# locuslab/lcp-physics

Measured on NVIDIA H100. Metric: LCP solves/sec (LCPFunction fwd+bwd, batch=4096 x 64 contacts, fp32), higher is better.
Workload: dtype f32 I/O and iterates; the condensed n x n KKT matrix is formed, factored and solved in f64

## Files before the change

lcp_physics_b200/csrc/lcp_condensed.cuh:

```cuda
#pragma once
#include "lcp_device.cuh"

namespace lcpb200 {
namespace cnd {

constexpr int NT = 256;
constexpr int UC = 8;
constexpr int CSMAX = 6;
constexpr int KS = 8;
constexpr int LMAX = 16;
constexpr int STATUS_UNSUPPORTED = -100;

struct CPlan {
  int ok;
  int n, m, e, N, NP, NS;
  int pcap;
  int wcap;
  int smem_bytes;
  int ctas_per_sm;
  int flags;
  int sbytes;
  int o_K, o_W, o_scr, o_bx, o_rdiag, o_Fd, o_Gd, o_As, o_x, o_rx, o_dx, o_qd, o_y, o_ry, o_dy,
      o_s, o_z, o_d, o_rz, o_ds, o_dz, o_rs2, o_red, o_rows, o_posof, o_clist, o_ccols, o_ncols, o_clcnt, o_misc;
};

__host__ __device__ inline size_t al16(size_t x) { return (x + 15) & ~(size_t)15; }
__host__ __device__ inline size_t scratch_bytes(int n, int m, int tsize) {
  return al16((size_t)2 * KS * m * 2) + al16((size_t)2 * KS * m * tsize) + al16((size_t)5 * m * 4) +
         al16((size_t)CSMAX * m * 2) + al16((size_t)8 * m * 4) + al16((size_t)LMAX * n * 2) + al16((size_t)n * 4) + 64;
}

inline size_t carve_plan(CPlan& P, int tsize) {
  size_t o = 0;
  const int n = P.n, m = P.m, e = P.e, NP = P.NP, pcap = P.pcap, wcap = P.wcap;
#define CND_TAKE(field, bytes) do { P.field = (int)o; o += al16((size_t)(bytes)); } while (0)
  size_t kb = (size_t)NP * NP * 8;
  if (scratch_bytes(n, m, tsize) > kb) kb = scratch_bytes(n, m, tsize);
  if ((size_t)8 * NP * 8 > kb) kb = (size_t)8 * NP * 8;
  { const size_t qn = (NP + 31) / 32, sl = (size_t)(NP / qn) * qn * qn * 32 * 8; if (sl > kb) kb = sl; }
  CND_TAKE(o_K, kb);
  CND_TAKE(o_W, (size_t)wcap * 8);
  CND_TAKE(o_scr, (size_t)pcap * 8);
  CND_TAKE(o_bx, (size_t)NP * 8);
  CND_TAKE(o_rdiag, (size_t)NP * 8);
  CND_TAKE(o_Fd, (size_t)wcap * tsize);
  CND_TAKE(o_Gd, (size_t)UC * pcap * tsize);
  CND_TAKE(o_As, (size_t)e * n * tsize);
  CND_TAKE(o_x, n * tsize); CND_TAKE(o_rx, n * tsize); CND_TAKE(o_dx, n * tsize); CND_TAKE(o_qd, n * tsize);
  CND_TAKE(o_y, e * tsize); CND_TAKE(o_ry, e * tsize); CND_TAKE(o_dy, e * tsize);
  CND_TAKE(o_s, m * tsize); CND_TAKE(o_z, m * tsize); CND_TAKE(o_d, m * tsize); CND_TAKE(o_rz, m * tsize);
  CND_TAKE(o_ds, m * tsize); CND_TAKE(o_dz, m * tsize); CND_TAKE(o_rs2, m * tsize);
  CND_TAKE(o_red, 192 * tsize);
  CND_TAKE(o_rows, pcap * 2);
  CND_TAKE(o_posof, m * 2);
  CND_TAKE(o_clist, LMAX * n * 2);
  CND_TAKE(o_ccols, UC * pcap);
  CND_TAKE(o_ncols, pcap);
  CND_TAKE(o_clcnt, n);
  CND_TAKE(o_misc, 16 * 4);
#undef CND_TAKE
  P.sbytes = 16 + (P.o_x - P.o_Fd) + (P.o_y - P.o_qd) + (P.o_misc - P.o_rows);
  return o;
}

extern __shared__ __align__(16) unsigned char cnd_smem[];

template <typename T>
struct CSmem {
  const CPlan& P;
  __device__ __forceinline__ explicit CSmem(const CPlan& p) : P(p) {}
#define CND_ACC(name, type) __device__ __forceinline__ type* name() const { return reinterpret_cast<type*>(cnd_smem + P.o_##name); }
  CND_ACC(K, double) CND_ACC(W, double) CND_ACC(scr, double) CND_ACC(bx, double) CND_ACC(rdiag, double)
  CND_ACC(Fd, T) CND_ACC(Gd, T) CND_ACC(As, T)
  CND_ACC(x, T) CND_ACC(rx, T) CND_ACC(dx, T) CND_ACC(qd, T) CND_ACC(y, T) CND_ACC(ry, T) CND_ACC(dy, T)
  CND_ACC(s, T) CND_ACC(z, T) CND_ACC(d, T) CND_ACC(rz, T) CND_ACC(ds, T) CND_ACC(dz, T) CND_ACC(rs2, T)
  CND_ACC(red, T)
  CND_ACC(rows, unsigned short) CND_ACC(posof, unsigned short) CND_ACC(clist, unsigned short)
  CND_ACC(ccols, unsigned char) CND_ACC(ncols, unsigned char) CND_ACC(clcnt, unsigned char)
  CND_ACC(misc, int)
#undef CND_ACC
};

struct Struct {
  int ncomp, cs;
  int sh;
  int m;
};

enum { CPH_STRUCT = 0, CPH_WINV, CPH_ASSEMBLE, CPH_LU, CPH_SOLVE_RHS, CPH_SOLVE_TRI, CPH_SOLVE_POST, CPH_RESID,
       CPH_STEP, CPH_GRADS, CPH_COUNT };
template <bool ON>
struct Prof {
  long long* p;
// ... 281 lines not shown
  T* ps = e_.p_s + (size_t)sc * n;
  T* hs = e_.h_s + (size_t)sc * P.m;
  int bad = 0;
  for (int j = tid; j < n; j += NT) {
    const int body = j / 3;
    const T q = (j - 3 * body == 0) ? inertia[body] : mass[body];
    S.qd()[j] = q;
    if (!(q != T(0) && isfinite((double)q))) bad |= 2;
    ps[j] = e_.mode == 0 ? q * v[j] + e_.dt * e_.fext[(size_t)sc * n + j] : T(0);
    cl_cnt[j] = 0;
  }
  for (int t = tid; t < e * n; t += NT) S.As()[t] = A[t];
  st.ncomp = nc; st.cs = cs; st.m = m;
  st.sh = 0;
  while ((1 << st.sh) < nc) ++st.sh;
  for (int t = tid; t < UC * pcap; t += NT) { S.Gd()[t] = T(0); S.ccols()[t] = 0; }
  for (int t = tid; t < nc * cs * cs; t += NT) S.Fd()[t] = T(0);
  __syncthreads();
  for (int c = tid; c < nc; c += NT) {
    const int b1 = tb1[c], b2 = tb2[c];
    if (b1 == b2 || b1 < 0 || b2 < 0 || b1 >= nb || b2 >= nb) { bad |= 1; continue; }
    const int lo = min(b1, b2), hi = max(b1, b2);
    const int o1 = b1 < b2 ? 0 : 3, o2 = 3 - o1;
#pragma unroll
    for (int q = 0; q < 3; ++q) {
      S.ccols()[q * pcap + c] = (unsigned char)(3 * lo + q);
      S.ccols()[(3 + q) * pcap + c] = (unsigned char)(3 * hi + q);
    }
    S.ncols()[c] = 6;
    const T nx = normal[2 * c], ny = normal[2 * c + 1];
    const T p1x = p1[2 * c], p1y = p1[2 * c + 1], p2x = p2[2 * c], p2y = p2[2 * c + 1];
    T r1[3], r2[3];
    contact_row<T>(p1x, p1y, p2x, p2y, nx, ny, r1, r2);
    const T jv = r1[0] * v[3 * b1] + r1[1] * v[3 * b1 + 1] + r1[2] * v[3 * b1 + 2] +
                 r2[0] * v[3 * b2] + r2[1] * v[3 * b2 + 1] + r2[2] * v[3 * b2 + 2];
    const T rc = e_.rest[(size_t)sc * ncs + c];
#pragma unroll
    for (int q = 0; q < 3; ++q) { S.Gd()[(size_t)(o1 + q) * pcap + c] = r1[q]; S.Gd()[(size_t)(o2 + q) * pcap + c] = r2[q]; }
    S.rows()[c] = (unsigned short)c;
    S.posof()[c] = (unsigned short)c;
    if (e_.mode == 0) {
      hs[c] = jv * rc;
      contact_row<T>(p1x, p1y, p2x, p2y, ny, -nx, r1, r2);
#pragma unroll
      for (int q = 0; q < 3; ++q) {
        S.Gd()[(size_t)(o1 + q) * pcap + nc + c] = r1[q];      S.Gd()[(size_t)(o2 + q) * pcap + nc + c] = r2[q];
        S.Gd()[(size_t)(o1 + q) * pcap + 2 * nc + c] = -r1[q]; S.Gd()[(size_t)(o2 + q) * pcap + 2 * nc + c] = -r2[q];
      }
      const int rw[4] = {c, nc + 2 * c, nc + 2 * c + 1, 3 * nc + c};
#pragma unroll
      for (int r = 0; r < 4; ++r) { S.rows()[r * nc + c] = (unsigned short)rw[r]; S.posof()[rw[r]] = (unsigned short)(r * nc + c); }
      hs[nc + 2 * c] = T(0); hs[nc + 2 * c + 1] = T(0); hs[3 * nc + c] = T(0);
      S.Fd()[(size_t)(1 * 4 + 3) * nc + c] = T(1);
      S.Fd()[(size_t)(2 * 4 + 3) * nc + c] = T(1);
      S.Fd()[(size_t)(3 * 4 + 0) * nc + c] = e_.mu[(size_t)sc * ncs + c];
      S.Fd()[(size_t)(3 * 4 + 1) * nc + c] = T(-1);
      S.Fd()[(size_t)(3 * 4 + 2) * nc + c] = T(-1);
    } else {
      hs[c] = jv + jv * -rc;
    }
    for (int q = 0; q < 6; ++q) {
      const int a = q < 3 ? 3 * lo + q : 3 * hi + q - 3;
      const int slot = atomicAdd(&cl_cnt[a], 1);
      if (slot < LMAX) cl_tmp[slot * n + a] = (unsigned short)(c * 8 + q); else bad |= 1;
    }
  }
  const int anybad = __syncthreads_or(bad);
  if (anybad & 2) { *singular = 1; return false; }
  if (anybad & 1) return false;
  for (int t = tid; t < n * LMAX; t += NT) {
    const int a = t % n, l = t / n, cnt = cl_cnt[a];
    if (l < cnt) {
      const int val = cl_tmp[l * n + a];
      int rank = 0;
      for (int u = 0; u < cnt; ++u) rank += (cl_tmp[u * n + a] < val);
      S.clist()[rank * n + a] = (unsigned short)val;
    }
    if (l == 0) S.clcnt()[a] = (unsigned char)cnt;
  }
  __syncthreads();
  return true;
}

__device__ __forceinline__ double rcp64_fast(double x) {
  double r;
  asm("rcp.approx.ftz.f64 %0, %1;" : "=d"(r) : "d"(x));
  const double ax = fabs(x);
  if (!(ax > 1e-290 && ax < 1e290)) return 1.0 / x;
  r = fma(r, fma(-x, r, 1.0), r);
  r = fma(r, fma(-x, r, 1.0), r);
  return r;
}

template <typename T, int CS>
__device__ __forceinline__ void comp_inverse(const CPlan& P, CSmem<T>& S, const Struct& st) {
  const int nc_ = st.ncomp;
  for (int c = threadIdx.x; c < nc_; c += NT) {
    double M[CS][CS];
#pragma unroll
    for (int r = 0; r < CS; ++r) {
      const int i = S.rows()[r * nc_ + c];
#pragma unroll
      for (int q = 0; q < CS; ++q) M[r][q] = (double)S.Fd()[(size_t)(r * CS + q) * nc_ + c];
      M[r][r] += (i == 0xFFFF) ? 1.0 : ((P.flags & 1) ? 1.0 / (double)S.d()[i] : (double)(T(1) / S.d()[i]));
    }
    unsigned swaps = 0;
    int bit = 0;
#pragma unroll
    for (int k = 0; k < CS; ++k) {
#pragma unroll
      for (int i = k + 1; i < CS; ++i) {
        const bool sw = fabs(M[i][k]) > fabs(M[k][k]);
        swaps |= (sw ? 1u : 0u) << bit;
        ++bit;
#pragma unroll
        for (int q = 0; q < CS; ++q) { const double u = M[k][q], w = M[i][q]; M[k][q] = sw ? w : u; M[i][q] = sw ? u : w; }
      }
      const double r = rcp64_fast(M[k][k]);
      M[k][k] = 1.0;
#pragma unroll
      for (int q = 0; q < CS; ++q) M[k][q] *= r;
#pragma unroll
      for (int i = 0; i < CS; ++i) {
        if (i == k) continue;
        const double f = M[i][k];
        M[i][k] = 0.0;
#pragma unroll
        for (int q = 0; q < CS; ++q) M[i][q] = fma(-f, M[k][q], M[i][q]);
      }
    }
#pragma unroll
    for (int k = CS - 1; k >= 0; --k) {
#pragma unroll
      for (int i = CS - 1; i > k; --i) {
        --bit;
        const bool sw = (swaps >> bit) & 1u;
#pragma unroll
        for (int q = 0; q < CS; ++q) { const double u = M[q][k], w = M[q][i]; M[q][k] = sw ? w : u; M[q][i] = sw ? u : w; }
      }
    }
#pragma unroll
    for (int r = 0; r < CS; ++r)
#pragma unroll
      for (int q = 0; q < CS; ++q) S.W()[(size_t)(r * CS + q) * nc_ + c] = M[r][q];
  }
}

template <typename T, int CS>
__device__ __forceinline__ void comp_apply(CSmem<T>& S, const Struct& st, bool trans = false) {
  const int nc_ = st.ncomp;
  const int npos = nc_ * CS;
  const int sh = st.sh, cmask = (1 << sh) - 1, tot = CS << sh;
  double val[4];
#pragma unroll
  for (int u = 0; u < 4; ++u) {
    const int t = threadIdx.x + u * NT, r = t >> sh, c = t & cmask;
    val[u] = 0.0;
    if (t < tot && c < nc_) {
      double a = 0.0;
#pragma unroll
      for (int q = 0; q < CS; ++q) a = fma(S.W()[(size_t)(trans ? (q * CS + r) : (r * CS + q)) * nc_ + c], S.scr()[q * nc_ + c], a);
      val[u] = a;
    }
  }
  __syncthreads();
#pragma unroll
  for (int u = 0; u < 4; ++u) {
    const int t = threadIdx.x + u * NT, r = t >> sh, c = t & cmask;
    if (t < tot && c < nc_) S.scr()[r * nc_ + c] = val[u];
  }
  (void)npos;
}

template <typename T, int NS, int CS>
__device__ __forceinline__ void assemble_K(const CPlan& P, CSmem<T>& S, const Struct& st) {
  const int nc_ = st.ncomp;
  constexpr int NP = 16 * NS;
  const int n = P.n, N = P.N, e = P.e, tid = threadIdx.x, pcap = P.pcap;
  double* K = S.K();
  {
    double2* K2 = reinterpret_cast<double2*>(K);
    for (int t = tid; t < NP * NP / 2; t += NT) K2[t] = make_double2(0.0, 0.0);
  }
  __syncthreads();
  for (int i = tid; i < NP; i += NT) K[(size_t)i * NP + i] = i < n ? (double)S.qd()[i] : (i < N ? 0.0 : 1.0);
  for (int t = tid; t < e * n; t += NT) {
    const int k = t / n, i = t - k * n;
    const double v = (double)S.As()[t];
    K[(size_t)(n + k) * NP + i] = v;
    K[(size_t)i * NP + n + k] = v;
  }
  __syncthreads();
  const int grp = tid >> 3, q2 = tid & 7;
  for (int a0 = 0; a0 < n; a0 += NT / 8) {
    const int a = a0 + grp;
    const int cnt = a < n ? (int)S.clcnt()[a] : 0;
    int mx = cnt;
    mx = max(mx, __shfl_xor_sync(FULL, mx, 8));
    mx = max(mx, __shfl_xor_sync(FULL, mx, 16));
    for (int l = 0; l < mx; ++l) {
      if (l < cnt) {
        const int cp = S.clist()[l * n + a], c = cp >> 3, p = cp & 7;
        if (q2 < (int)S.ncols()[c]) {
          double acc = 0.0;
#pragma unroll
          for (int q = 0; q < CS; ++q) {
            double u = 0.0;
#pragma unroll
            for (int r = 0; r < CS; ++r)
              u = fma((double)S.Gd()[(size_t)p * pcap + r * nc_ + c], S.W()[(size_t)(r * CS + q) * nc_ + c], u);
            acc = fma(u, (double)S.Gd()[(size_t)q2 * pcap + q * nc_ + c], acc);
          }
          K[(size_t)S.ccols()[q2 * pcap + c] * NP + a] += acc;
        }
      }
      __syncwarp();
    }
  }
  __syncthreads();
}

template <int NS, int B0>
__device__ __forceinline__ void lu_phase(double (&a)[NS][NS], int o_buf, int o_rdiag, int& step, int ti, int tj) {
  constexpr int NP = 16 * NS;
  constexpr int L = NS - B0;
  constexpr int CW = (L <= 4) ? L : 3;
  double* const rdiag = reinterpret_cast<double*>(cnd_smem + o_rdiag);
#pragma unroll 1
  for (int kk = 0; kk < 16; kk += 2) {
    const int k = 16 * B0 + kk;
    double2* const U2 = reinterpret_cast<double2*>(cnd_smem + o_buf) + (size_t)(step & 1) * 2 * NP;
    double2* const C2 = U2 + NP;
    ++step;
    {
      const int sr = ti - kk, sc = tj - kk;
      if ((unsigned)sr < 2u) {
        double* dst = reinterpret_cast<double*>(U2) + sr;
#pragma unroll
        for (int c = B0; c < NS; ++c) dst[2 * (16 * c + tj)] = a[B0][c];
      }
      if ((unsigned)sc < 2u) {
        double* dst = reinterpret_cast<double*>(C2) + sc;
#pragma unroll
        for (int r = B0; r < NS; ++r) dst[2 * (16 * r + ti)] = a[r][B0];
      }
    }
    __syncthreads();
    const double2 pk = U2[k], pk1 = U2[k + 1];
    const double p01 = pk1.x;
    const double r0 = rcp64_fast(pk.x);
    const double r1 = pk.x * rcp64_fast(fma(pk.x, pk1.y, -(pk.y * p01)));
    const double l10 = pk.y * r0;
    if ((ti | tj) == 0) { rdiag[k] = r0; rdiag[k + 1] = r1; }
#pragma unroll
    for (int cg = B0; cg < NS; cg += CW) {
      double w0[CW], w1[CW];
#pragma unroll
      for (int q = 0; q < CW; ++q) {
        const int c = cg + q;
        if (c < NS) {
          const double2 u = U2[16 * c + tj];
          const double x1 = fma(-l10, u.x, u.y);
          w0[q] = (c == B0 && !(tj > kk)) ? 0.0 : u.x;
          w1[q] = (c == B0 && !(tj > kk + 1)) ? 0.0 : x1;
        }
      }
#pragma unroll
      for (int r = B0; r < NS; ++r) {
        const double2 cc = C2[16 * r + ti];
        double m0 = cc.x * r0;
        double m1 = fma(-m0, p01, cc.y) * r1;
        if (r == B0) {
          m0 = (ti > kk) ? m0 : 0.0;
          m1 = (ti > kk + 1) ? m1 : 0.0;
        }
#pragma unroll
        for (int q = 0; q < CW; ++q) {
          const int c = cg + q;
          if (c < NS) a[r][c] = fma(-m1, w1[q], fma(-m0, w0[q], a[r][c]));
        }
      }
    }
  }
}

template <int NS, int B0>
struct LuPhases {
  static __device__ __forceinline__ void run(double (&a)[NS][NS], int o_buf, int o_rdiag, int& step, int ti, int tj) {
    lu_phase<NS, B0>(a, o_buf, o_rdiag, step, ti, tj);
    LuPhases<NS, B0 + 1>::run(a, o_buf, o_rdiag, step, ti, tj);
  }
};
template <int NS>
struct LuPhases<NS, NS> {
  static __device__ __forceinline__ void run(double (&)[NS][NS], int, int, int&, int, int) {}
};

template <int NS> struct SolveLayout {
  static constexpr int NP = 16 * NS;
  static constexpr int QN = (NP + 31) / 32;
  static constexpr int ROUNDS = NP / QN;
  static constexpr size_t BYTES = (size_t)ROUNDS * QN * QN * 32 * 8;
};

template <int NS>
__device__ __noinline__ void factor_K(int o_K, int o_rdiag, bool trans) {
  constexpr int NP = 16 * NS, QN = SolveLayout<NS>::QN;
  int tid_;
  asm volatile("mov.u32 %0, %%tid.x;" : "=r"(tid_));
  const int ti = tid_ & 15, tj = tid_ >> 4;
  double* const K = reinterpret_cast<double*>(cnd_smem + o_K);
  double* const rdiag = reinterpret_cast<double*>(cnd_smem + o_rdiag);
  double a[NS][NS];
#pragma unroll
  for (int c = 0; c < NS; ++c)
#pragma unroll
    for (int r = 0; r < NS; ++r) a[r][c] = K[(size_t)(16 * c + tj) * NP + 16 * r + ti];
  __syncthreads();
  int step = 0;
  LuPhases<NS, 0>::run(a, o_K, o_rdiag, step, ti, tj);
  __syncthreads();
  int rowpart[NS];
  double rrow[NS];
#pragma unroll
  for (int r = 0; r < NS; ++r) {
    const int i = 16 * r + ti;
    rowpart[r] = trans ? (i / QN) * QN * QN * 32 + (i % QN) * 32 : (i % QN) * QN * 32 + i / QN;
    rrow[r] = rdiag[i];
  }
#pragma unroll
  for (int c = 0; c < NS; ++c) {
    const int j = 16 * c + tj;
    const double rj = rdiag[j];
    const int colpart = trans ? (j % QN) * QN * 32 + j / QN : (j / QN) * QN * QN * 32 + (j % QN) * 32;
#pragma unroll
    for (int r = 0; r < NS; ++r) {
      const int i = 16 * r + ti;
      K[colpart + rowpart[r]] = (i != j) ? a[r][c] * (trans ? rrow[r] : rj) : a[r][c];
    }
  }
  __syncthreads();
}

template <int QN>
struct SolveCoef {
  double dg[QN * QN];
  double rw[QN * QN];
};

template <int QN>
__device__ __forceinline__ void solve_load(SolveCoef<QN>& c, const double* blk, int r, int lane) {
#pragma unroll
  for (int t = 0; t < QN * QN; ++t) { c.dg[t] = blk[t * 32 + r]; c.rw[t] = blk[t * 32 + lane]; }
}

template <int QN>
__device__ __forceinline__ void solve_round_fwd(double (&y)[QN], const SolveCoef<QN>& c, int r, int lane) {
  double v[QN];
#pragma unroll
  for (int q = 0; q < QN; ++q) v[q] = __shfl_sync(FULL, y[q], r);
#pragma unroll
  for (int q = 0; q < QN; ++q)
#pragma unroll
    for (int qp = q + 1; qp < QN; ++qp) v[qp] = fma(-c.dg[qp * QN + q], v[q], v[qp]);
  const bool below = lane > r, own = lane == r;
#pragma unroll
  for (int qp = 0; qp < QN; ++qp) {
    double t = y[qp];
#pragma unroll
    for (int q = 0; q < QN; ++q) t = fma(-c.rw[qp * QN + q], v[q], t);
    y[qp] = below ? t : (own ? v[qp] : y[qp]);
  }
}

template <int QN>
__device__ __forceinline__ void solve_round_bwd(double (&y)[QN], const SolveCoef<QN>& c, int r, int lane) {
  double v[QN];
#pragma unroll
  for (int q = 0; q < QN; ++q) v[q] = __shfl_sync(FULL, y[q], r);
#pragma unroll
  for (int q = QN - 1; q >= 0; --q)
#pragma unroll
    for (int qp = q - 1; qp >= 0; --qp) v[qp] = fma(-c.dg[qp * QN + q], v[q], v[qp]);
  const bool above = lane < r, own = lane == r;
#pragma unroll
  for (int qp = 0; qp < QN; ++qp) {
    double t = y[qp];
#pragma unroll
    for (int q = QN - 1; q >= 0; --q) t = fma(-c.rw[qp * QN + q], v[q], t);
    y[qp] = above ? t : (own ? v[qp] : y[qp]);
  }
}

template <int NS>
__device__ __noinline__ void solve_warp(int o_K, int o_rdiag, int o_bx) {
  constexpr int NP = 16 * NS, QN = SolveLayout<NS>::QN, ROUNDS = SolveLayout<NS>::ROUNDS;
  constexpr int STRIDE = QN * QN * 32;
  static_assert(ROUNDS % 2 == 0, "the software pipeline handles two rounds per trip");
  const int lane = threadIdx.x & 31;
  const double* const S = reinterpret_cast<const double*>(cnd_smem + o_K);
  const double* const rdiag = reinterpret_cast<const double*>(cnd_smem + o_rdiag);
  double* const bx = reinterpret_cast<double*>(cnd_smem + o_bx);
  double y[QN];
#pragma unroll
  for (int q = 0; q < QN; ++q) y[q] = (QN * lane + q < NP) ? bx[QN * lane + q] : 0.0;
  SolveCoef<QN> c0, c1;
  solve_load<QN>(c0, S, 0, lane);
#pragma unroll 1
  for (int r = 0; r < ROUNDS; r += 2) {
    solve_load<QN>(c1, S + (size_t)(r + 1) * STRIDE, r + 1, lane);
    solve_round_fwd<QN>(y, c0, r, lane);
    const int rn = (r + 2 < ROUNDS) ? r + 2 : ROUNDS - 1;
    solve_load<QN>(c0, S + (size_t)rn * STRIDE, rn, lane);
    solve_round_fwd<QN>(y, c1, r + 1, lane);
  }
#pragma unroll 1
  for (int r = ROUNDS - 1; r > 0; r -= 2) {
    solve_load<QN>(c1, S + (size_t)(r - 1) * STRIDE, r - 1, lane);
    solve_round_bwd<QN>(y, c0, r, lane);
    const int rn = (r - 2 >= 0) ? r - 2 : 0;
    solve_load<QN>(c0, S + (size_t)rn * STRIDE, rn, lane);
    solve_round_bwd<QN>(y, c1, r - 1, lane);
  }
#pragma unroll
  for (int q = 0; q < QN; ++q) {
    const int i = QN * lane + q;
    if (i < NP) bx[i] = y[q] * rdiag[i];
  }
}

template <typename T, int CS, int NS, typename PF>
__device__ __noinline__ void solve_kkt(const CPlan& P, CSmem<T> S, Struct st, PF& pf, const T* rx,
                                       const T* rs, const T* rz, const T* ry, T* dx, T* ds, T* dz, T* dy,
                                       bool trans = false) {
  const int nc_ = st.ncomp;
  const int n = P.n, e = P.e, N = P.N, NP = P.NP, tid = threadIdx.x, pcap = P.pcap;
  const int npos = st.ncomp * CS;
  for (int p = tid; p < npos; p += NT) {
    const int i = S.rows()[p];
    double t = 0.0;
    if (i != 0xFFFF) t = (P.flags & 2) ? ((double)(rz ? rz[i] : T(0)) - (double)rs[i] / (double)S.d()[i]) : (double)((rz ? rz[i] : T(0)) - rs[i] / S.d()[i]);
    S.scr()[p] = t;
  }
  __syncthreads();
  comp_apply<T, CS>(S, st, trans);
  __syncthreads();
  for (int a = tid; a < NP; a += NT) {
    double acc = 0.0;
    if (a < n) {
      const int cnt = S.clcnt()[a];
      for (int l = 0; l < cnt; ++l) {
        const int cp = S.clist()[l * n + a], c = cp >> 3, p = cp & 7;
#pragma unroll
        for (int r = 0; r < CS; ++r) acc = fma((double)S.Gd()[(size_t)p * pcap + r * nc_ + c], S.scr()[r * nc_ + c], acc);
      }
      acc = -(double)(rx ? rx[a] : T(0)) - acc;
    } else if (a < N) {
      acc = -(double)(ry ? ry[a - n] : T(0));
    }
    S.bx()[a] = acc;
  }
  __syncthreads();
  pf.lap(CPH_SOLVE_RHS);
  if (tid < 32) solve_warp<NS>(P.o_K, P.o_rdiag, P.o_bx);
  __syncthreads();
  pf.lap(CPH_SOLVE_TRI);
  for (int tt = tid; tt < (CS << st.sh); tt += NT) {
    const int c = tt & ((1 << st.sh) - 1);
    if (c >= nc_) continue;
    const int p = (tt >> st.sh) * nc_ + c;
    const int i = S.rows()[p];
    double t = 0.0;
    if (i != 0xFFFF) {
      const int nc = S.ncols()[c];
      t = (P.flags & 2) ? ((double)(rz ? rz[i] : T(0)) - (double)rs[i] / (double)S.d()[i]) : (double)((rz ? rz[i] : T(0)) - rs[i] / S.d()[i]);
      for (int q = 0; q < nc; ++q) t = fma((double)S.Gd()[(size_t)q * pcap + p], S.bx()[S.ccols()[q * pcap + c]], t);
    }
    S.scr()[p] = t;
  }
  __syncthreads();
  comp_apply<T, CS>(S, st, trans);
  __syncthreads();
  for (int p = tid; p < npos; p += NT) {
    const int i = S.rows()[p];
    if (i == 0xFFFF) continue;
    const T wz = (T)S.scr()[p];
    const T rsi = rs[i];
    dz[i] = wz;
    ds[i] = (-rsi - wz) / S.d()[i];
  }
  for (int a = tid; a < n; a += NT) dx[a] = (T)S.bx()[a];
  for (int k = tid; k < e; k += NT) dy[k] = (T)S.bx()[n + k];
  __syncthreads();
  pf.lap(CPH_SOLVE_POST);
}

template <typename T, int NS, int CS, typename PF>
__device__ __noinline__ void factor_kkt(const CPlan& P, CSmem<T> S, Struct st, PF& pf, bool trans = false) {
  comp_inverse<T, CS>(P, S, st);
  __syncthreads();
  pf.lap(CPH_WINV);
  assemble_K<T, NS, CS>(P, S, st);
  pf.lap(CPH_ASSEMBLE);
  factor_K<NS>(P.o_K, P.o_rdiag, trans);
  pf.lap(CPH_LU);
}

template <typename T>
__device__ __forceinline__ void get_steps(const T* z, const T* dz, const T* s, const T* ds, int m, T* red, T& step_z,
                                          T& step_s) {
  const T NEG_INF = -INFINITY, POS_INF = INFINITY;
  T mx[2] = {NEG_INF, NEG_INF};
  T mn[2] = {POS_INF, POS_INF};
  T any[2] = {T(0), T(0)};
  for (int i = threadIdx.x; i < m; i += NT) {
    const T az = -z[i] / dz[i], as = -s[i] / ds[i];
    mx[0] = nan_max(mx[0], az);
    mx[1] = nan_max(mx[1], as);
    if (dz[i] > T(0)) any[0] = T(1); else mn[0] = nan_min(mn[0], az);
    if (ds[i] > T(0)) any[1] = T(1); else mn[1] = nan_min(mn[1], as);
  }
  T v[6] = {mx[0], mx[1], -mn[0], -mn[1], any[0], any[1]};
  block_reduce<T, 6>(v, OpMax(), NEG_INF, red);
  const T fz = (v[0] > T(1)) ? v[0] : T(1);
  const T fs = (v[1] > T(1)) ? v[1] : T(1);
  step_z = (v[4] > T(0)) ? nan_min(-v[2], fz) : -v[2];
  step_s = (v[5] > T(0)) ? nan_min(-v[3], fs) : -v[3];
}

template <typename T>
struct CFwdArgs {
  CPlan P;
  int B;
  const T *Q, *p, *G, *h, *A, *b, *F;
  T *zhat, *nu, *lam, *slack, *resid;
  int *status, *iters;
  T eps;
  int not_improved_lim, max_iter;
  long long* prof;
  EngineSoA<T> soa;
  unsigned char* ssave;
};

template <typename T>
struct CBwdArgs {
  CPlan P;
  int B;
  const T *Q, *G, *A, *F;
  const T *zhat, *nu, *lam, *slack, *g;
  T *dQ, *dp, *dG, *dh, *dA, *db, *dF;
  int* done;
  const int* only;
  unsigned flags;
  const unsigned char* sload;
  EngineSoA<T> soa;
  T *dmass, *dinertia, *dv, *dfext, *dnormal, *dp1, *dp2, *dmu, *drest;
  long long* prof;
};

__device__ __forceinline__ void copy16(unsigned char* dst, const unsigned char* src, int bytes) {
  const uint4* s4 = reinterpret_cast<const uint4*>(src);
  uint4* d4 = reinterpret_cast<uint4*>(dst);
  for (int i = threadIdx.x; i < (bytes >> 4); i += NT) d4[i] = s4[i];
}

__device__ __forceinline__ void save_structure(const CPlan& P, const Struct& st, bool ok, unsigned char* dst) {
  if (threadIdx.x == 0) *reinterpret_cast<int4*>(dst) = make_int4(ok ? st.ncomp : -1, st.cs, st.sh, st.m);
  if (!ok) return;
  const int c1 = P.o_x - P.o_Fd, c2 = P.o_y - P.o_qd, c3 = P.o_misc - P.o_rows;
  copy16(dst + 16, cnd_smem + P.o_Fd, c1);
  copy16(dst + 16 + c1, cnd_smem + P.o_qd, c2);
  copy16(dst + 16 + c1 + c2, cnd_smem + P.o_rows, c3);
}

__device__ __forceinline__ bool load_structure(const CPlan& P, Struct& st, const unsigned char* src) {
  const int4 hd = *reinterpret_cast<const int4*>(src);
  st.ncomp = hd.x; st.cs = hd.y; st.sh = hd.z; st.m = hd.w;
  if (hd.x < 0) return false;
  const int c1 = P.o_x - P.o_Fd, c2 = P.o_y - P.o_qd, c3 = P.o_misc - P.o_rows;
  copy16(cnd_smem + P.o_Fd, src + 16, c1);
  copy16(cnd_smem + P.o_qd, src + 16 + c1, c2);
  copy16(cnd_smem + P.o_rows, src + 16 + c1 + c2, c3);
  return true;
}

template <typename T>
struct SzResid { T sz, resid; };
// ... 111 lines not shown
  solve_kkt<T, CS, NS>(P, S, st, pf, S.rx(), S.rs2(), S.rz(), P.e > 0 ? S.ry() : nullptr, S.x(), S.s(), S.z(), S.y());
  if (m == 0) {
    fwd_store_best<T>(a, S, 0, sc);
    if (threadIdx.x == 0) { a.status[sc] = 2; a.iters[sc] = 0; if (a.resid) a.resid[sc] = T(0); }
    return;
  }
  {
    const int tid = threadIdx.x;
    T mn[2] = {INFINITY, INFINITY};
    for (int i = tid; i < m; i += NT) { mn[0] = nan_min(mn[0], S.s()[i]); mn[1] = nan_min(mn[1], S.z()[i]); }
    block_reduce<T, 2>(mn, OpMin(), (T)INFINITY, S.red());
    for (int i = tid; i < m; i += NT) {
      if (mn[0] <= T(0)) S.s()[i] -= mn[0] - T(1);
      if (mn[1] <= T(0)) S.z()[i] -= mn[1] - T(1);
    }
    __syncthreads();
  }

  T best = nan("");
  bool have_best = false;
  int not_improved = 0, status = 0, it = 0;
  for (it = 0; it < a.max_iter; ++it) {
    const SzResid<T> r = fwd_residuals<T, CS>(a, S, st, sc);
    pf.lap(CPH_RESID);
    const T mu = fabs(r.sz / T(m));

    bool improved;
    if (!have_best) { improved = true; have_best = true; not_improved = 0; }
    else { improved = r.resid < best; not_improved = improved ? 0 : not_improved + 1; }
    if (improved) {
      best = r.resid;
      fwd_store_best<T>(a, S, m, sc);
    }
    if (not_improved == a.not_improved_lim) { status = 1; ++it; break; }
    if (best < a.eps) { status = 2; ++it; break; }
    if (mu > T(1e100)) { status = 3; ++it; break; }

    for (int i = threadIdx.x; i < m; i += NT) S.d()[i] = S.z()[i] / S.s()[i];
    __syncthreads();
    factor_kkt<T, NS, CS>(P, S, st, pf);

    solve_kkt<T, CS, NS>(P, S, st, pf, S.rx(), S.z(), S.rz(), P.e > 0 ? S.ry() : nullptr, S.dx(), S.ds(), S.dz(), S.dy());
    fwd_centering<T>(S, m, mu, r.sz);
    pf.lap(CPH_STEP);
    solve_kkt<T, CS, NS>(P, S, st, pf, nullptr, S.rs2(), nullptr, nullptr, S.rx(), S.rz(), S.rs2(), S.ry());
    fwd_step<T>(P, S, m);
    pf.lap(CPH_STEP);
  }
  if (threadIdx.x == 0) { a.status[sc] = status; a.iters[sc] = it; if (a.resid) a.resid[sc] = best; }
}

template <typename T, int NS, bool PROF>
__global__ void __launch_bounds__(NT, (NS <= 6) ? 2 : 1) cond_forward_kernel(const __grid_constant__ CFwdArgs<T> a) {
  const CPlan& P = a.P;
  CSmem<T> S(P);
  const int n = P.n, m = P.m, e = P.e, tid = threadIdx.x;
  __shared__ int singular_s;
  const T NANV = nan("");
  Prof<PROF> pf(PROF ? a.prof + (size_t)blockIdx.x * CPH_COUNT : nullptr);
  for (int sc = blockIdx.x; sc < a.B; sc += gridDim.x) {
    if (tid == 0) singular_s = 0;
    __syncthreads();
    pf.start();
    Struct st;
    const bool ok = a.soa.mass
        ? build_structure_soa<T>(P, S, st, a.soa, sc, e > 0 ? a.A + (size_t)sc * e * n : nullptr, &singular_s)
        : build_structure<T>(P, S, st, a.Q + (size_t)sc * n * n, a.G + (size_t)sc * m * n,
                             e > 0 ? a.A + (size_t)sc * e * n : nullptr, a.F + (size_t)sc * m * m, &singular_s);
    __syncthreads();
    if (a.ssave) save_structure(P, st, ok, a.ssave + (size_t)sc * P.sbytes);
    pf.lap(CPH_STRUCT);
    if (!ok) {
      if (singular_s) {
        for (int i = tid; i < n; i += NT) a.zhat[(size_t)sc * n + i] = NANV;
        for (int i = tid; i < m; i += NT) { a.lam[(size_t)sc * m + i] = NANV; a.slack[(size_t)sc * m + i] = NANV; }
        for (int i = tid; i < e; i += NT) a.nu[(size_t)sc * e + i] = NANV;
        if (tid == 0) { a.status[sc] = -1; a.iters[sc] = 0; if (a.resid) a.resid[sc] = NANV; }
      } else if (tid == 0) {
        a.status[sc] = STATUS_UNSUPPORTED;
      }
      __syncthreads();
      continue;
    }
    switch (st.cs) {
      case 1: forward_scene<T, NS, 1>(a, S, st, pf, sc); break;
      case 2: forward_scene<T, NS, 2>(a, S, st, pf, sc); break;
      case 3: forward_scene<T, NS, 3>(a, S, st, pf, sc); break;
      case 4: forward_scene<T, NS, 4>(a, S, st, pf, sc); break;
      case 5: forward_scene<T, NS, 5>(a, S, st, pf, sc); break;
      default: forward_scene<T, NS, 6>(a, S, st, pf, sc); break;
    }
    __syncthreads();
  }
}

template <typename T, typename F>
__device__ __forceinline__ void write_outer(T* __restrict__ o, int rows, int cols, F f) {
  constexpr int V = 16 / (int)sizeof(T);
  const int tid = threadIdx.x;
  if (cols % V == 0 && (reinterpret_cast<size_t>(o) & 15) == 0) {
    const int cv = cols / V, total = rows * cv;
    const int di = NT / cv, dj = NT - di * cv;
    int i = tid / cv, jv = tid - i * cv;
    for (int t = tid; t < total; t += NT) {
      const int j = jv * V;
      if (V == 4) {
        float4 w;
        w.x = (float)f(i, j); w.y = (float)f(i, j + 1); w.z = (float)f(i, j + 2); w.w = (float)f(i, j + 3);
        reinterpret_cast<float4*>(o)[t] = w;
      } else {
        double2 w;
        w.x = (double)f(i, j); w.y = (double)f(i, j + 1);
        reinterpret_cast<double2*>(o)[t] = w;
      }
      i += di; jv += dj;
      if (jv >= cv) { jv -= cv; ++i; }
    }
  } else {
    int i = tid / cols, j = tid - i * cols;
    const int di = NT / cols, dj = NT - di * cols;
    for (size_t t = tid; t < (size_t)rows * cols; t += NT) {
      o[t] = f(i, j);
      i += di; j += dj;
      if (j >= cols) { j -= cols; ++i; }
    }
  }
}

template <typename T, int NS, int CS, typename PF>
__device__ __forceinline__ void backward_scene(const CBwdArgs<T>& a, CSmem<T>& S, const Struct& st, PF& pf, int sc) {
  const CPlan& P = a.P;
  const int n = P.n, m = st.m, e = P.e, tid = threadIdx.x;
  const T* zh = a.zhat + (size_t)sc * n;
  const T* lam = a.lam + (size_t)sc * P.m;
  const T* slk = a.slack + (size_t)sc * P.m;
  const T* nu = e > 0 ? a.nu + (size_t)sc * e : nullptr;
  for (int i = tid; i < n; i += NT) { S.x()[i] = zh[i]; S.rx()[i] = a.g[(size_t)sc * n + i]; }
  for (int i = tid; i < m; i += NT) {
    T d = lam[i] / slk[i];
    if (sizeof(T) == 8) d = d > T(1e10) ? T(1e10) : (d < T(1e-10) ? T(1e-10) : d);
    S.z()[i] = lam[i]; S.s()[i] = slk[i]; S.d()[i] = d; S.rs2()[i] = T(0);
  }
  for (int i = tid; i < e; i += NT) S.y()[i] = nu[i];
  __syncthreads();
  const bool exact = (a.flags & 1u) != 0;
  factor_kkt<T, NS, CS>(P, S, st, pf, exact);
  solve_kkt<T, CS, NS>(P, S, st, pf, S.rx(), S.rs2(), nullptr, nullptr, S.dx(), S.ds(), S.dz(), S.dy(), exact);
  const T* dx = S.dx(); const T* dlam = S.dz(); const T* dnu = S.dy();
  if (a.soa.mass) {
    const EngineSoA<T>& E = a.soa;
    const int nc = st.ncomp, nb = E.nb, ncs = E.nc;
    const int32_t* tb1 = E.b1 + (E.nc_s ? (size_t)sc * ncs : 0);
    const int32_t* tb2 = E.b2 + (E.nc_s ? (size_t)sc * ncs : 0);
    const T* v = E.v + (size_t)sc * n;
    const T* zh_ = S.x(); const T* lm = S.z();
    for (int c = tid; c < ncs; c += NT) {
      const size_t ic = (size_t)sc * ncs + c;
      if (c >= nc) {
        if (a.dnormal) { a.dnormal[ic * 2] = 0; a.dnormal[ic * 2 + 1] = 0; }
        if (a.dp1) { a.dp1[ic * 2] = 0; a.dp1[ic * 2 + 1] = 0; }
        if (a.dp2) { a.dp2[ic * 2] = 0; a.dp2[ic * 2 + 1] = 0; }
        if (a.drest) a.drest[ic] = 0;
        if (a.dmu) a.dmu[ic] = 0;
        continue;
      }
      const T nx = E.normal[ic * 2], ny = E.normal[ic * 2 + 1];
// ... 34 lines not shown
      if (a.dmu) a.dmu[ic] = E.mode == 0 ? -(dlam[3 * nc + c] * lm[c]) : T(0);
    }
    for (int j = tid; j < n; j += NT) {
      const int body = j / 3, comp = j - 3 * body;
      const T md = comp == 0 ? E.inertia[(size_t)sc * nb + body] : E.mass[(size_t)sc * nb + body];
      const T dpj = E.mode == 0 ? dx[j] : T(0);
      if (a.dfext) a.dfext[(size_t)sc * n + j] = E.dt * dpj;
      if (a.dv) {
        T acc = md * dpj;
        const int cnt = S.clcnt()[j];
        for (int l = 0; l < cnt; ++l) {
          const int cp = S.clist()[l * n + j], c = cp >> 3, pslot = cp & 7;
          const T hs_ = E.mode == 0 ? E.rest[(size_t)sc * ncs + c] : (T(1) - E.rest[(size_t)sc * ncs + c]);
          acc += -dlam[c] * hs_ * S.Gd()[(size_t)pslot * P.pcap + c];
        }
        a.dv[(size_t)sc * n + j] = acc;
      }
      const T dqjj = dx[j] * zh_[j];
      if (comp == 0 && a.dinertia) a.dinertia[(size_t)sc * nb + body] = dqjj + dpj * v[j];
    }
    __syncthreads();
    for (int body = tid; body < nb; body += NT) {
      if (!a.dmass) break;
      T acc = 0;
      for (int comp = 1; comp < 3; ++comp) {
        const int j = 3 * body + comp;
        acc += dx[j] * zh_[j] + (E.mode == 0 ? dx[j] : T(0)) * v[j];
      }
      a.dmass[(size_t)sc * nb + body] = acc;
    }
    if (a.db && e > 0) for (int i = tid; i < e; i += NT) a.db[(size_t)sc * e + i] = -dnu[i];
    if (a.dA && e > 0) {
      T* o = a.dA + (size_t)sc * e * n;
      for (int i = 0; i < e; ++i)
        for (int j = tid; j < n; j += NT) o[(size_t)i * n + j] = dnu[i] * S.x()[j] + S.y()[i] * dx[j];
    }
    if (tid == 0 && a.done) a.done[sc] = 1;
    __syncthreads();
    pf.lap(CPH_GRADS);
    return;
  }
  if (a.dp) for (int i = tid; i < n; i += NT) a.dp[(size_t)sc * n + i] = dx[i];
  if (a.dh) for (int i = tid; i < m; i += NT) a.dh[(size_t)sc * m + i] = -dlam[i];
  if (a.db && e > 0) for (int i = tid; i < e; i += NT) a.db[(size_t)sc * e + i] = -dnu[i];
  if (a.dG)
    write_outer<T>(a.dG + (size_t)sc * m * n, m, n, [&](int i, int j) { return dlam[i] * S.x()[j] + S.z()[i] * dx[j]; });
  if (a.dF)
    write_outer<T>(a.dF + (size_t)sc * m * m, m, m, [&](int i, int j) { return -(dlam[i] * S.z()[j]); });
  if (a.dA && e > 0)
    write_outer<T>(a.dA + (size_t)sc * e * n, e, n, [&](int i, int j) { return dnu[i] * S.x()[j] + S.y()[i] * dx[j]; });
  if (a.dQ)
    write_outer<T>(a.dQ + (size_t)sc * n * n, n, n, [&](int i, int j) { return T(0.5) * (dx[i] * S.x()[j] + S.x()[i] * dx[j]); });
  if (tid == 0 && a.done) a.done[sc] = 1;
  __syncthreads();
  pf.lap(CPH_GRADS);
}

template <typename T, int NS, bool PROF>
__global__ void __launch_bounds__(NT, (NS <= 6) ? 2 : 1) cond_backward_kernel(const __grid_constant__ CBwdArgs<T> a) {
  const CPlan& P = a.P;
  CSmem<T> S(P);
  const int n = P.n, m = P.m, e = P.e, tid = threadIdx.x;
  __shared__ int singular_s;
  Prof<PROF> pf(PROF ? a.prof + (size_t)blockIdx.x * CPH_COUNT : nullptr);
  for (int sc = blockIdx.x; sc < a.B; sc += gridDim.x) {
    if (a.only && !a.only[sc]) continue;
    if (tid == 0) singular_s = 0;
    __syncthreads();
    pf.start();
    Struct st;
    const bool ok = a.soa.mass
        ? build_structure_soa<T>(P, S, st, a.soa, sc, e > 0 ? a.A + (size_t)sc * e * n : nullptr, &singular_s)
        : a.sload
              ? load_structure(P, st, a.sload + (size_t)sc * P.sbytes)
              : build_structure<T>(P, S, st, a.Q + (size_t)sc * n * n, a.G + (size_t)sc * m * n,
                                   e > 0 ? a.A + (size_t)sc * e * n : nullptr, a.F + (size_t)sc * m * m, &singular_s);
    __syncthreads();
    pf.lap(CPH_STRUCT);
    if (!ok) {
      if (tid == 0 && a.done) a.done[sc] = 0;
      __syncthreads();
      continue;
    }
    switch (st.cs) {
      case 1: backward_scene<T, NS, 1>(a, S, st, pf, sc); break;
      case 2: backward_scene<T, NS, 2>(a, S, st, pf, sc); break;
      case 3: backward_scene<T, NS, 3>(a, S, st, pf, sc); break;
      case 4: backward_scene<T, NS, 4>(a, S, st, pf, sc); break;
      case 5: backward_scene<T, NS, 5>(a, S, st, pf, sc); break;
      default: backward_scene<T, NS, 6>(a, S, st, pf, sc); break;
    }
    __syncthreads();
  }
}

}
}
```

Baseline: 266,500.

## Add block-banded LU path for condensed KKT when coupling stays within band

Before each scene, scans the component column lists to check whether all couplings fall within a block bandwidth of 2 (16-row tiles), and sets a shared flag. When the flag is set, the register-tiled LU factorisation stores and updates only the band of blocks, skipping fill-in updates outside it and cutting register footprint. Falls back to the dense LU when equality constraints exist or a dense flag is set. This adds a per-scene scan and a second template instantiation, which grows code size, and relies on the band check being correct for fill-in.

```diff
diff --git a/lcp_physics_b200/csrc/lcp_condensed.cuh b/lcp_physics_b200/csrc/lcp_condensed.cuh
--- a/lcp_physics_b200/csrc/lcp_condensed.cuh
+++ b/lcp_physics_b200/csrc/lcp_condensed.cuh
@@ -9,6 +9,9 @@
 constexpr int CSMAX = 6;
 constexpr int KS = 8;
 constexpr int LMAX = 16;
+constexpr int LU_BW = 2;
+constexpr int MISC_BAND_LU = 4;
+constexpr int CFLAG_DENSE_LU = 4;
 constexpr int STATUS_UNSUPPORTED = -100;
 
 struct CPlan {
@@ -456,6 +459,17 @@
   return true;
 }
 
+template <typename T>
+__device__ __noinline__ void mark_band_lu(const CPlan& P, CSmem<T> S, Struct st) {
+  int wide = P.e > 0 || (P.flags & CFLAG_DENSE_LU);
+  for (int c = threadIdx.x; c < st.ncomp; c += NT) {
+    const int nc = S.ncols()[c];
+    if (nc > 0 && (S.ccols()[(nc - 1) * P.pcap + c] >> 4) - (S.ccols()[c] >> 4) > LU_BW) wide = 1;
+  }
+  wide = __syncthreads_or(wide);
+  if (threadIdx.x == 0) S.misc()[MISC_BAND_LU] = !wide;
+}
+
 __device__ __forceinline__ double rcp64_fast(double x) {
   double r;
   asm("rcp.approx.ftz.f64 %0, %1;" : "=d"(r) : "d"(x));
@@ -594,10 +608,22 @@
   __syncthreads();
 }
 
-template <int NS, int B0>
-__device__ __forceinline__ void lu_phase(double (&a)[NS][NS], int o_buf, int o_rdiag, int& step, int ti, int tj) {
+template <int NS, int BW>
+struct LuBand {
+  static constexpr bool DENSE = BW >= NS - 1;
+  static constexpr int W = DENSE ? NS : 2 * BW + 1;
+  static __device__ __forceinline__ constexpr bool in(int r, int c) { return DENSE || (r - c <= BW && c - r <= BW); }
+  static __device__ __forceinline__ constexpr int col(int r, int c) { return DENSE ? c : c - r + BW; }
+  static __host__ __device__ constexpr int end(int b0) { return DENSE || b0 + BW + 1 > NS ? NS : b0 + BW + 1; }
+};
+
+template <int NS, int BW, int B0>
+__device__ __forceinline__ void lu_phase(double (&a)[NS][LuBand<NS, BW>::W], int o_buf, int o_rdiag, int& step, int ti,
+                                         int tj) {
+  using Bd = LuBand<NS, BW>;
   constexpr int NP = 16 * NS;
-  constexpr int L = NS - B0;
+  constexpr int E = Bd::end(B0);
+  constexpr int L = E - B0;
   constexpr int CW = (L <= 4) ? L : 3;
   double* const rdiag = reinterpret_cast<double*>(cnd_smem + o_rdiag);
 #pragma unroll 1
@@ -611,12 +637,12 @@
       if ((unsigned)sr < 2u) {
         double* dst = reinterpret_cast<double*>(U2) + sr;
 #pragma unroll
-        for (int c = B0; c < NS; ++c) dst[2 * (16 * c + tj)] = a[B0][c];
+        for (int c = B0; c < E; ++c) dst[2 * (16 * c + tj)] = a[B0][Bd::col(B0, c)];
       }
       if ((unsigned)sc < 2u) {
         double* dst = reinterpret_cast<double*>(C2) + sc;
 #pragma unroll
-        for (int r = B0; r < NS; ++r) dst[2 * (16 * r + ti)] = a[r][B0];
+        for (int r = B0; r < E; ++r) dst[2 * (16 * r + ti)] = a[r][Bd::col(r, B0)];
       }
     }
     __syncthreads();
@@ -627,12 +653,12 @@
     const double l10 = pk.y * r0;
     if ((ti | tj) == 0) { rdiag[k] = r0; rdiag[k + 1] = r1; }
 #pragma unroll
-    for (int cg = B0; cg < NS; cg += CW) {
+    for (int cg = B0; cg < E; cg += CW) {
       double w0[CW], w1[CW];
 #pragma unroll
       for (int q = 0; q < CW; ++q) {
         const int c = cg + q;
-        if (c < NS) {
+        if (c < E) {
           const double2 u = U2[16 * c + tj];
           const double x1 = fma(-l10, u.x, u.y);
           w0[q] = (c == B0 && !(tj > kk)) ? 0.0 : u.x;
@@ -640,7 +666,7 @@
         }
       }
 #pragma unroll
-      for (int r = B0; r < NS; ++r) {
+      for (int r = B0; r < E; ++r) {
         const double2 cc = C2[16 * r + ti];
         double m0 = cc.x * r0;
         double m1 = fma(-m0, p01, cc.y) * r1;
@@ -651,23 +677,24 @@
 #pragma unroll
         for (int q = 0; q < CW; ++q) {
           const int c = cg + q;
-          if (c < NS) a[r][c] = fma(-m1, w1[q], fma(-m0, w0[q], a[r][c]));
+          if (c < E) a[r][Bd::col(r, c)] = fma(-m1, w1[q], fma(-m0, w0[q], a[r][Bd::col(r, c)]));
         }
       }
     }
   }
 }
 
-template <int NS, int B0>
+template <int NS, int BW, int B0>
 struct LuPhases {
-  static __device__ __forceinline__ void run(double (&a)[NS][NS], int o_buf, int o_rdiag, int& step, int ti, int tj) {
-    lu_phase<NS, B0>(a, o_buf, o_rdiag, step, ti, tj);
-    LuPhases<NS, B0 + 1>::run(a, o_buf, o_rdiag, step, ti, tj);
+  static __device__ __forceinline__ void run(double (&a)[NS][LuBand<NS, BW>::W], int o_buf, int o_rdiag, int& step, int ti,
+                                             int tj) {
+    lu_phase<NS, BW, B0>(a, o_buf, o_rdiag, step, ti, tj);
+    LuPhases<NS, BW, B0 + 1>::run(a, o_buf, o_rdiag, step, ti, tj);
   }
 };
-template <int NS>
-struct LuPhases<NS, NS> {
-  static __device__ __forceinline__ void run(double (&)[NS][NS], int, int, int&, int, int) {}
+template <int NS, int BW>
+struct LuPhases<NS, BW, NS> {
+  static __device__ __forceinline__ void run(double (&)[NS][LuBand<NS, BW>::W], int, int, int&, int, int) {}
 };
 
 template <int NS> struct SolveLayout {
@@ -677,22 +704,24 @@
   static constexpr size_t BYTES = (size_t)ROUNDS * QN * QN * 32 * 8;
 };
 
-template <int NS>
-__device__ __noinline__ void factor_K(int o_K, int o_rdiag, bool trans) {
+template <int NS, int BW>
+__device__ __forceinline__ void factor_K_body(int o_K, int o_rdiag, bool trans) {
+  using Bd = LuBand<NS, BW>;
   constexpr int NP = 16 * NS, QN = SolveLayout<NS>::QN;
   int tid_;
   asm volatile("mov.u32 %0, %%tid.x;" : "=r"(tid_));
   const int ti = tid_ & 15, tj = tid_ >> 4;
   double* const K = reinterpret_cast<double*>(cnd_smem + o_K);
   double* const rdiag = reinterpret_cast<double*>(cnd_smem + o_rdiag);
-  double a[NS][NS];
+  double a[NS][Bd::W];
 #pragma unroll
   for (int c = 0; c < NS; ++c)
 #pragma unroll
-    for (int r = 0; r < NS; ++r) a[r][c] = K[(size_t)(16 * c + tj) * NP + 16 * r + ti];
+    for (int r = 0; r < NS; ++r)
+      if (Bd::in(r, c)) a[r][Bd::col(r, c)] = K[(size_t)(16 * c + tj) * NP + 16 * r + ti];
   __syncthreads();
   int step = 0;
-  LuPhases<NS, 0>::run(a, o_K, o_rdiag, step, ti, tj);
+  LuPhases<NS, BW, 0>::run(a, o_K, o_rdiag, step, ti, tj);
   __syncthreads();
   int rowpart[NS];
   double rrow[NS];
@@ -710,10 +739,22 @@
 #pragma unroll
     for (int r = 0; r < NS; ++r) {
       const int i = 16 * r + ti;
-      K[colpart + rowpart[r]] = (i != j) ? a[r][c] * (trans ? rrow[r] : rj) : a[r][c];
-    }
-  }
-  __syncthreads();
+      const double v = Bd::in(r, c) ? a[r][Bd::col(r, c)] : 0.0;
+      K[colpart + rowpart[r]] = (i != j) ? v * (trans ? rrow[r] : rj) : v;
+    }
+  }
+  __syncthreads();
+}
+
+template <int NS>
+__device__ __noinline__ void factor_K(int o_K, int o_rdiag, bool trans, bool band) {
+  if constexpr (LU_BW < NS - 1) {
+    if (band) {
+      factor_K_body<NS, LU_BW>(o_K, o_rdiag, trans);
+      return;
+    }
+  }
+  factor_K_body<NS, NS - 1>(o_K, o_rdiag, trans);
 }
 
 template <int QN>
@@ -876,7 +917,8 @@
   pf.lap(CPH_WINV);
   assemble_K<T, NS, CS>(P, S, st);
   pf.lap(CPH_ASSEMBLE);
-  factor_K<NS>(P.o_K, P.o_rdiag, trans);
+  if constexpr (LU_BW < NS - 1) factor_K<NS>(P.o_K, P.o_rdiag, trans, S.misc()[MISC_BAND_LU] != 0);
+  else factor_K<NS>(P.o_K, P.o_rdiag, trans, false);
   pf.lap(CPH_LU);
 }
 
@@ -1154,6 +1196,7 @@
       __syncthreads();
       continue;
     }
+    if constexpr (LU_BW < NS - 1) mark_band_lu<T>(P, S, st);
     switch (st.cs) {
       case 1: forward_scene<T, NS, 1>(a, S, st, pf, sc); break;
       case 2: forward_scene<T, NS, 2>(a, S, st, pf, sc); break;
@@ -1354,6 +1397,7 @@
       __syncthreads();
       continue;
     }
+    if constexpr (LU_BW < NS - 1) mark_band_lu<T>(P, S, st);
     switch (st.cs) {
       case 1: backward_scene<T, NS, 1>(a, S, st, pf, sc); break;
       case 2: backward_scene<T, NS, 2>(a, S, st, pf, sc); break;
```

Result: faster. 306,000, median of 6 (+14.8%).
